# DanieleTeni/Online-Non-Linear-Centroidal-MPC-with-stability-Guarantees-for-Robust-Locomotion-of-Legged-Robots-

Hardware: AMD Instinct MI355X
Metric: centroidal-MPC solves/sec, N=20 horizon (higher is better)
Workload: dtype f64

## Files before the change

### __graft_entry__.py

```python
import os
import sys

ROOT = os.path.dirname(os.path.abspath(__file__))
if ROOT not in sys.path:
    sys.path.insert(0, ROOT)


def build():
    import build as _b
    _b.build_hip()
    _b.build_oracle()
    _b.build_emu()
    _b.build_emu_gain()
    _b.build_emu_consts()
    _b.build_emu_reuse()
    _b.build_emu_reuse(reuse=False)
    _b.build_device_unit()
    _b.build_tools()
    import ctypes
    import torch
    import cmpc_amd
    from cmpc_amd import capi
    lib = ctypes.CDLL(capi.LIB_PATH)
    for sym in capi.SYMBOLS:
        getattr(lib, sym)


def smoke():
    import numpy as np
    import torch
    import cmpc_amd
    from cmpc_amd import workloads as wl
    from cmpc_amd.solver import BatchedCentroidalMPC
    from oracle import oracle_lib as ol

    assert torch.cuda.is_available(), "smoke() needs a GPU"
    spec, rec = wl.make_workload("perturbed", B=8, N=10, scale=0.25)
    solver = BatchedCentroidalMPC(spec, device="cuda:0")
    out, status, iters, kkt = solver.solve(torch.from_numpy(rec).to("cuda:0"))
# ... 18 lines not shown
```

### build.py

```python
import os
import subprocess
import sys

ROOT = os.path.dirname(os.path.abspath(__file__))
PKG = os.path.join(ROOT, "online-non-linear-centroidal-mpc-with-stability-guarantees-for-robust-locomotion-of-legged-robots-_amd")


def _newer(target, sources):
    if not os.path.exists(target):
        return True
    t = os.path.getmtime(target)
    return any(os.path.getmtime(s) > t for s in sources)


CSRC = os.path.join(PKG, "csrc")
KERNEL_DEPS = [os.path.join(CSRC, "cmpc_kernel.hpp"), os.path.join(CSRC, "cmpc_lds_asm.hpp"), os.path.join(CSRC, "cmpc_wave.hpp"),
               os.path.join(ROOT, "include", "cmpc.h")]
DEVICE_DEPS = [os.path.join(CSRC, "cmpc_hip.hip"), os.path.join(CSRC, "wbc_qp.hip")] + KERNEL_DEPS + [
    os.path.join(CSRC, "cmpc_order_fit.h"), os.path.join(ROOT, "include", "cmpc_wbc.h")]
EMU_DIR = os.path.join(ROOT, "tests", "emu")


def _hipcc_lib(out, defines=(), force=False, verbose=False):
    if force or _newer(out, DEVICE_DEPS):
# ... 5 lines not shown

def _emu_lib(src, out, defines=(), force=False):
    src, out = os.path.join(EMU_DIR, src), os.path.join(EMU_DIR, out)
    if force or _newer(out, [src, os.path.join(EMU_DIR, "cmpc_emu.cpp")] + KERNEL_DEPS):
        subprocess.check_call(["g++", "-O2", "-std=c++17", "-mfma", "-ffp-contract=off", "-fPIC", "-shared", "-pthread"]
                              + ["-D" + d for d in defines] + ["-o", out, src])
    return out


def build_hip(force=False, verbose=False):
    return _hipcc_lib(os.path.join(PKG, "libcmpc_amd.so"), force=force, verbose=verbose)


def build_hip_profile(force=False):
    return _hipcc_lib(os.path.join(ROOT, "tools", "libcmpc_amd_prof.so"), ["CMPC_PROFILE"], force)


def build_hip_dev(force=False):
    return _hipcc_lib(os.path.join(ROOT, "tools", "libcmpc_amd_dev.so"), ["CMPC_DEV_KNOBS"], force)


def build_hip_no_reuse(force=False, profile=False):
    return _hipcc_lib(os.path.join(ROOT, "tools", "libcmpc_amd_noreuse_prof.so" if profile else "libcmpc_amd_noreuse.so"),
                      ["CMPC_NO_EVAL_REUSE"] + (["CMPC_PROFILE"] if profile else []), force)


def build_oracle(force=False):
    out = os.path.join(ROOT, "oracle", "libcmpc_oracle.so")
    deps = [os.path.join(ROOT, "oracle", "cmpc_oracle.c"), os.path.join(ROOT, "include", "cmpc.h")]
    if force or _newer(out, deps):
        subprocess.check_call(["make", "-C", os.path.join(ROOT, "oracle"), "-B", "libcmpc_oracle.so"],
                              stdout=subprocess.DEVNULL)
    return out


def build_emu(force=False):
    return _emu_lib("cmpc_emu.cpp", "libcmpc_emu.so", force=force)


def build_emu_gain(force=False):
    return _emu_lib("cmpc_emu_gain.cpp", "libcmpc_emu_gain.so", force=force)


def build_emu_consts(force=False):
    return _emu_lib("cmpc_emu_consts.cpp", "libcmpc_emu_consts.so", force=force)


def build_emu_reuse(force=False, reuse=True):
    return _emu_lib("cmpc_emu_reuse.cpp", "libcmpc_emu_reuse.so" if reuse else "libcmpc_emu_noreuse.so",
                    [] if reuse else ["CMPC_NO_EVAL_REUSE"], force)


def build_device_unit(force=False):
    src = os.path.join(ROOT, "tests", "gpu_unit", "cmpc_device_unit.hip")
    out = os.path.join(ROOT, "tests", "gpu_unit", "libcmpc_device_unit.so")
    if force or _newer(out, [src] + KERNEL_DEPS):
        subprocess.check_call(["hipcc", "--offload-arch=gfx950", "-O3", "-std=c++17", "-fPIC", "-shared", "-o", out, src])
    return out


def build_tools(force=False):
    outs = []
    for name in ("hbm_calib", "lds_b128_repro"):
        src = os.path.join(ROOT, "tools", "ubench", name + ".hip")
        out = os.path.join(ROOT, "tools", "ubench", name)
        if force or _newer(out, [src]):
            r = subprocess.run(["hipcc", "--offload-arch=gfx950", "-O3", "-o", out, src], capture_output=True, text=True)
            if r.returncode != 0:
                print(f"build_tools: {name} failed to compile (profiling scripts that need it will not run)\n{r.stderr}",
                      file=sys.stderr)
                continue
        outs.append(out)
    return outs


if __name__ == "__main__":
    force = "--force" in sys.argv
    print(build_hip(force, verbose="-v" in sys.argv))
    print(build_oracle(force))
    print(build_emu(force))
    print(build_emu_gain(force))
    print(build_emu_consts(force))
    print(build_emu_reuse(force))
    print(build_emu_reuse(force, reuse=False))
    print(build_device_unit(force))
    print(build_tools(force))
```

### online-non-linear-centroidal-mpc-with-stability-guarantees-for-robust-locomotion-of-legged-robots-_amd/csrc/cmpc_kernel.hpp

```cpp
#pragma once
#include "../../include/cmpc.h"
#include <math.h>
#include <utility>
#ifdef CMPC_HOST_EMU
#include <cstdio>
#include <cstdlib>
#endif

#ifndef CMPC_HOST_EMU
#include <hip/hip_runtime.h>
#define CMPC_DEV __device__ __forceinline__
#define CMPC_LANE ((int)threadIdx.x)
#define CMPC_SYNC() asm volatile("s_waitcnt lgkmcnt(0)" ::: "memory")
#define CMPC_SYNC_GLOBAL() __syncthreads()
#define CMPC_SYNC_WG() asm volatile("s_waitcnt lgkmcnt(0)\n\ts_barrier" ::: "memory")
#define CMPC_WAVE_ID() ((int)__builtin_amdgcn_readfirstlane((int)threadIdx.x >> 6))
static __device__ __forceinline__ double cmpc_bcast(double v, int src) {
  union { double d; int i[2]; } u; u.d = v;
  u.i[0] = __builtin_amdgcn_readlane(u.i[0], src);
  u.i[1] = __builtin_amdgcn_readlane(u.i[1], src);
  return u.d;
}
#define CMPC_BCAST(v, src) cmpc_bcast((v), (src))
typedef double cmpc_v4d __attribute__((ext_vector_type(4)));
// ... 11 lines not shown
#else
#define SPD(field) (EVAL_REUSE ? cmpc_fresh(CMPC_SPEC_OR_ROW(field)) : CMPC_SPEC_OR_ROW(field))
#endif
typedef const double __attribute__((address_space(4))) *cmpc_crow_t;
#define CMPC_CROW(p) ((cmpc_crow_t)(p))
static __device__ __forceinline__ cmpc_crow_t cmpc_fresh_row(cmpc_crow_t r) { asm volatile("" : "+s"(r)); return r; }
#define CMPC_ROW_AT(r, i) (cmpc_fresh_row(r)[i])
static __device__ __forceinline__ double cmpc_uniform_d(double v) {
  union { double d; int i[2]; } u; u.d = v;
  int lo, hi;
  asm("s_nop 0\n\tv_readfirstlane_b32 %0, %2\n\tv_readfirstlane_b32 %1, %3\n\ts_nop 1" : "=s"(lo), "=s"(hi) : "v"(u.i[0]), "v"(u.i[1]));
  u.i[0] = lo; u.i[1] = hi;
  return u.d;
}
#ifdef CMPC_NO_UNIFORM_D
#define CMPC_UNIFORM_D(x) (x)
#else
#define CMPC_UNIFORM_D(x) cmpc_uniform_d(x)
#endif
#define CMPC_SCHED_FENCE() __builtin_amdgcn_sched_barrier(0)
#define CMPC_RELANE(x) do { (x) = (int)__builtin_amdgcn_mbcnt_hi(~0u, __builtin_amdgcn_mbcnt_lo(~0u, 0u)) + lane_base; } while (0)
#define CMPC_SYNC_WAVE(w) CMPC_SYNC()
#define CMPC_FENCE_WAVE(w) asm volatile("s_waitcnt vmcnt(0) lgkmcnt(0)" ::: "memory")
#endif
#ifdef CMPC_HOST_EMU
#define CMPC_SYNC_WAVE(w) emu_barrier_wait(&emu_wave_barrier[(w)])
#define CMPC_FENCE_WAVE(w) emu_barrier_wait(&emu_wave_barrier[(w)])
#define CMPC_SYNC_WG() emu_barrier_wait(&emu_barrier)
#endif
#ifndef CMPC_RELANE
#define CMPC_RELANE(x) do { } while (0)
#define SPD(field) CMPC_SPEC_OR_ROW(field)
typedef const double *cmpc_crow_t;
#define CMPC_CROW(p) ((cmpc_crow_t)(p))
#define CMPC_ROW_AT(r, i) ((r)[i])
#define CMPC_FRESH_D(x) (x)
#define CMPC_UNIFORM_D(x) (x)
#endif
#define CMPC_CIDX(field) ((int)((__builtin_offsetof(cmpc_spec, field) - __builtin_offsetof(cmpc_spec, delta)) / sizeof(double)))
#define CMPC_SPEC_OR_ROW(field) (CONSTS ? CMPC_ROW_AT(crow, CMPC_CIDX(field)) : sp.field)
static_assert(CMPC_CIDX(relax) == CMPC_NCONST - 1 && CMPC_CIDX(box[2]) == 13 && __builtin_offsetof(cmpc_spec, tol) == __builtin_offsetof(cmpc_spec, relax) + sizeof(double),
              "the row of per-instance constants is the block of cmpc_spec from delta to relax");
#define CMPC_FMA(x, y, z) __builtin_fma((x), (y), (z))
#ifndef CMPC_OPAQUE_D
#define CMPC_OPAQUE_D(x) do { } while (0)
#endif
#ifndef CMPC_UNIFORM_INT
#define CMPC_UNIFORM_INT(x) (x)
#endif
#ifndef CMPC_OPAQUE_S
#define CMPC_OPAQUE_S(x) do { } while (0)
#endif

#if defined(CMPC_PROFILE) && !defined(CMPC_HOST_EMU)
static __device__ __forceinline__ constexpr int cmpc_retry_class(int slot) {
  return (slot == 11 || slot == 12 || slot == 26 || slot == 0) ? 31
       : (slot == 24 || slot == 25) ? 32
       : (slot == 27) ? 34
       : 33;
}
#define CMPC_TICK(slot) do { long long now_ = clock64(); tprof[slot] += now_ - tlast; \
    if (prof_retry) tprof[cmpc_retry_class(slot)] += now_ - tlast; \
    tlast = now_; } while (0)
#define CMPC_TICK_RESET() do { tlast = clock64(); } while (0)
#define CMPC_RETRY_STAT(slot, n) do { tprof[slot] += (n); } while (0)
#define CMPC_RETRY_MARK(on) do { prof_retry = (on); } while (0)
#define CMPC_RETRY_TRACK 1
#else
#define CMPC_TICK(slot) do { } while (0)
#define CMPC_TICK_RESET() do { } while (0)
#define CMPC_RETRY_MARK(on) do { } while (0)
#define CMPC_RETRY_TRACK 0
#endif
#ifndef CMPC_RETRY_STAT
#define CMPC_RETRY_STAT(slot, n) do { } while (0)
#endif
#define CMPC_NPROF 36

namespace cmpc {

struct KArgs {
  cmpc_spec sp;
  int B;
  const double *recs;
  const double *warm;
  const double *state_in;
  double *state_out;
  double *out;
  int32_t *status;
  int32_t *iters;
  double *kkt;
  double *scratch;
  size_t scratch_stride;
  long long *prof;
  double tol_acc, tol_tenth;
};

enum { R_LYAP = 0, R_CZ = 1, R_HWC = 2, R_BOX = 3, R_FRIC = 15 };
// ... 108 lines not shown
  using S = Sizes<4, 1>;
#ifdef CMPC_NO_GT_FIRST
  static constexpr bool GT = true, GT_FIRST = false;
#else
  static constexpr bool GT = true, GT_FIRST = !PIPE;
#endif
  static constexpr int oM = 0;
  static constexpr int oP = oM + S::NTRI + (S::NTRI & 1);
  static constexpr bool P_PACKED = true;
  static constexpr int P_DOUBLES = S::NPT + (S::NPT & 1);
  static constexpr int DUMPN = 16;
  static constexpr int MISCN = 52;
  static constexpr int oXN1 = oP + P_DOUBLES;
  static constexpr int oSR = oXN1 + S::NXA;
  static constexpr int oSRP = oSR + 20;
  static constexpr int oHDR = oSRP + 20;
  static constexpr int oH0 = oHDR + 24;
  static constexpr int oH1 = oH0 + S::NZ;
  static constexpr int oPC1 = oH1 + S::NZ;
  static constexpr int oPC = oPC1 + S::NXA;
  static constexpr int oRED = oPC + S::NXA;
  static constexpr int oCOLD = oRED + 4;
  static constexpr int oDUMP = oCOLD + 8;
  static constexpr int oXK = oDUMP + DUMPN + ((oDUMP + DUMPN) & 1);
  static constexpr int oUK = oXK + S::NXA;
  static constexpr int oLAMK = oUK + S::NU;
  static constexpr int oLAMN = oLAMK + S::NXA;
  static constexpr int oUPX = oLAMN + S::NXA;
  static constexpr int oSK = oUPX + S::NU;
  static constexpr int oZK = oSK + S::NI;
  static constexpr int oVDV = oZK + S::NI;
  static constexpr int oMISC = oVDV + 3 * S::NF;
  static constexpr int oLATE = oMISC + MISCN;
  static constexpr int LATE_DOUBLES = S::NZ + 4 * S::NI;
  static constexpr int oAL = GT_FIRST ? oP : oLATE;
  static constexpr int oGK = oAL + S::NZ;
  static constexpr int oW0 = oGK + S::NI;
  static constexpr int oW1 = oW0 + S::NI;
  static constexpr int oW2 = oW1 + S::NI;
  static_assert(!GT_FIRST || LATE_DOUBLES <= P_DOUBLES, "the late evaluation vectors fit the dead P region");
  static constexpr int oGH = GT_FIRST ? oM : oLATE + LATE_DOUBLES;
  static constexpr int oBV = oGH + 3 * S::NZ;
  static constexpr int oVR = GT_FIRST ? oBV + S::NXA : oAL;
  static constexpr int oEND = GT_FIRST ? oLATE : oBV + S::NXA;
  static constexpr int oTV = oSK;
  static constexpr int oTV2 = oXK;
// ... 60 lines not shown
    ok = ok && v < INFINITY && v > -INFINITY && (positive ? v > 0.0 : (gain || v >= 0.0));
  }
  return ok;
}

template <int NV, int NW = 1, bool PIPE = false, bool GAIN = false, bool CONSTS = false> struct Solver {
  using D = Dims<NV, NW, PIPE>;
  static constexpr int XCH_DU = 16, XCH_DOUBLES = XCH_DU + 2 * D::NU;
  static_assert(!PIPE || XCH_DOUBLES <= D::P_DOUBLES, "the exchange words fit in the unused P region of the second image");
  static constexpr int XCH_AT = D::LDS_DOUBLES + D::oP;
  static_assert(!PIPE || NW == 1, "the pipelined pair runs the one-wave solver");
  static_assert(!PIPE || (D::oUB + 64 <= D::oBV && D::oUB >= D::oXN1 + D::NXA && !D::GT_FIRST),
                "pair_vectors reads BV / writes XN1 of the image the Riccati wave is working in");
  static constexpr int NF = D::NF, NU = D::NU, NXA = D::NXA, NZ = D::NZ, NI = D::NI, NH = D::NH, WS = D::WS;
  static_assert(NW == 1 || NU <= 64, "the input rows (pivot chains, substitutions) live in the first wave");
#ifdef CMPC_NO_EVAL_REUSE
  static constexpr bool EVAL_REUSE = false;
#else
  static constexpr bool EVAL_REUSE = NV == 4 && NW == 1 && !PIPE && !GAIN && D::GT_FIRST;
#endif
  static constexpr bool RETRY_TRACK_POSSIBLE = NV == 4 && NW == 1 && !PIPE && !GAIN;
  static constexpr int ER_AT = 256;
  static_assert(!RETRY_TRACK_POSSIBLE || (ER_AT >= 3 * NZ + NXA + 3 * NF && ER_AT + 6 * WS <= D::NTRI), "the parked error measures fit the M region");
  static constexpr bool RETRY_TRACK = EVAL_REUSE || (CMPC_RETRY_TRACK && NV == 4 && NW == 1 && !PIPE && !GAIN);

  const KArgs &ka;
  const cmpc_spec &sp;
  double *lds;
  double *ldsR;
  int lane_base = 0;
  GArr gs;
  GArr rec;
  int N, lane;
  int wv = 0;
  GArr gx, glam, gdx, glamn, gu, gdu, gupx, gsl, gz, gds, gdz;
  int lr[NH][6];
  double lg[NH][6];
  double piv_min = PIV_MIN;
  GArr st_in{nullptr};
  long long tprof[CMPC_NPROF] = {0, 0, 0, 0, 0, 0, 0, 0, 0, 0, 0, 0, 0, 0, 0, 0, 0, 0, 0, 0, 0, 0, 0, 0, 0, 0, 0, 0, 0, 0, 0, 0, 0, 0, 0, 0}, tlast = 0;
  bool prof_retry = false;
  double *gain_out = nullptr;
  GArr gbuf{nullptr};
  bool gain_sweep = false;
  cmpc_crow_t crow = nullptr;

  CMPC_DEV Solver(const KArgs &a, double *l, double *g, const double *r)
// ... 28 lines not shown
    else {
#ifdef CMPC_HOST_EMU
      CMPC_SYNC();
#else
      if constexpr (NW == 1) CMPC_SYNC(); else CMPC_SYNC_WG();
#endif
    }
  }
  CMPC_DEV void gsync() const {
    if constexpr (PIPE) { CMPC_FENCE_WAVE(wv); } else { CMPC_SYNC_GLOBAL(); }
  }
  CMPC_DEV void pair_sync() const { if constexpr (PIPE) { CMPC_SYNC_GLOBAL(); } }
  CMPC_DEV bool first_wave() const { return NW == 1 || wv == 0; }

  CMPC_DEV double gam_k(int k, int f) const { return (k == N) ? L(D::oHDR + 22 + f) : L(D::oSR + 17 + f); }
  CMPC_DEV double gam_km1(int f) const { return L(D::oSRP + 17 + f); }
  CMPC_DEV void vert_local(int j, double &vx, double &vy) const {
    const double Lh = SPD(foot_length) * 0.5, Wh = SPD(foot_width) * 0.5;
    const double cx[8] = {Lh, Lh, -Lh, -Lh, Lh, 0.0, -Lh, 0.0};
    const double cy[8] = {Wh, -Wh, -Wh, Wh, 0.0, -Wh, 0.0, Wh};
    vx = cx[j]; vy = cy[j];
  }

  CMPC_DEV void load_stage(int k) {
    static_assert(NXA <= 64 && NU <= 64, "one lane per state / input component");
    constexpr int NIH = (NI + WS - 1) / WS;
    const bool in = k < N;
    const int kn = in ? k + 1 : k, ku = in ? k : N - 1, kp = (k >= 1) ? k - 1 : 0;
    const int ix = (lane < NXA) ? lane : 0, iu = (lane < NU) ? lane : 0, ir = (lane < 19) ? lane : 0;
    const double x0 = gx[k * NXA + ix], x1 = gx[kn * NXA + ix];
    const double u0 = gu[ku * NU + iu], up = gupx[ku * NU + iu];
    const double r0 = rec[24 + 19 * ku + ir], r1 = rec[24 + 19 * kp + ir], hd = rec[(lane < 24) ? lane : 0];
    double sv[NIH], zv[NIH];
    const double l0 = glam[k * NXA + ix], l1 = glam[kn * NXA + ix];
    {
#pragma unroll
      for (int h = 0; h < NIH; ++h) {
        const int r = lane + WS * h, rc = (r < NI) ? r : 0;
        sv[h] = gsl[k * NI + rc]; zv[h] = gz[k * NI + rc];
      }
    }
    if (lane < NXA) {
      L(D::oXK + lane) = x0; L(D::oXN1 + lane) = in ? x1 : 0.0;
      L(D::oLAMK + lane) = l0; L(D::oLAMN + lane) = in ? l1 : 0.0;
    }
    if (lane < NU) { L(D::oUK + lane) = in ? u0 : 0.0; L(D::oUPX + lane) = in ? up : 0.0; }
    {
#pragma unroll
      for (int h = 0; h < NIH; ++h) {
        const int r = lane + WS * h;
        if (r < NI) { L(D::oSK + r) = sv[h]; L(D::oZK + r) = zv[h]; }
      }
    }
    if (lane < 19) { L(D::oSR + lane) = in ? r0 : 0.0; L(D::oSRP + lane) = (k >= 1) ? r1 : 0.0; }
    if (lane < 24) L(D::oHDR + lane) = hd;
    sync();
  }

  CMPC_DEV void stage_geometry(int k) {
    const double d = SPD(delta), m = L(D::oHDR + 20);
    double *tq = &L(D::oH0), *yw = &L(D::oH0 + 3 * NF), *qq = &L(D::oH0 + 6 * NF);
    static_assert(7 * NF <= 2 * NZ, "vertex products fit the H0/H1 block");
    if (lane < NF) {
      const int f = lane / NV, j = lane % NV;
      const double yaw = L(D::oXK + 12 + 4 * f);
      const double px = L(D::oXK + 13 + 4 * f), py = L(D::oXK + 14 + 4 * f), pz = L(D::oXK + 15 + 4 * f);
      const double cx = L(D::oXK + 0), cy = L(D::oXK + 1), cz = L(D::oXK + 2);
      const double fx = L(D::oUK + 3 * lane), fy = L(D::oUK + 3 * lane + 1), fz = L(D::oUK + 3 * lane + 2);
      const double p0 = d * L(D::oLAMN + 6), p1 = d * L(D::oLAMN + 7), p2 = d * L(D::oLAMN + 8);
      const double cs = cos(yaw), sn = sin(yaw);
      double vx, vy; vert_local(j, vx, vy);
      const double rvx = cs * vx - sn * vy, rvy = sn * vx + cs * vy;
      const double dvx = -sn * vx - cs * vy, dvy = cs * vx - sn * vy;
      const double rx = px + rvx - cx, ry = py + rvy - cy, rz = pz - cz;
      L(D::oVDV + 3 * lane + 0) = dvx; L(D::oVDV + 3 * lane + 1) = dvy; L(D::oVDV + 3 * lane + 2) = 0.0;
      L(D::oVR + 3 * lane + 0) = rx; L(D::oVR + 3 * lane + 1) = ry; L(D::oVR + 3 * lane + 2) = rz;
      tq[3 * lane + 0] = ry * fz - rz * fy; tq[3 * lane + 1] = rz * fx - rx * fz; tq[3 * lane + 2] = rx * fy - ry * fx;
      yw[3 * lane + 0] = dvy * fz; yw[3 * lane + 1] = -dvx * fz; yw[3 * lane + 2] = dvx * fy - dvy * fx;
      qq[lane] = p0 * (-rvy * fz) + p1 * (rvx * fz) + p2 * (-rvx * fy + rvy * fx);
// ... 893 lines not shown
      const double a = (b0 + b1) + (b2 + b3);
      L(D::oXN1 + lane) = R(D::oPC + lane) + a;
      st[D::gB + lane] = L(D::oBV + lane);
    }
  }
  CMPC_DEV double list_dot(int h, const double *v) const {
    double a = 0.0;
#pragma unroll
    for (int n = 0; n < 6; ++n) a = CMPC_FMA(lg[h][n], v[lr[h][n]], a);
    CMPC_OPAQUE_D(a);
    return a;
  }

  CMPC_DEV void eval_stage(int k, double mu, double reg, double wz, double x0n2, Err &er, bool init, bool reuse_ = false) {
    const bool reuse = EVAL_REUSE && reuse_;
    CMPC_RELANE(lane); CMPC_OPAQUE(lane);
    if constexpr (EVAL_REUSE) { CMPC_OPAQUE_S(k); }
    double re_h0 = 0.0, re_h1 = 0.0, re_al = 0.0, re_w0 = 0.0;
    if (reuse) {
      const GArr sk = stage(k); const unsigned re = restage(k);
      const int cz = (lane < NZ) ? lane : 0, ci = (lane < NI) ? lane : 0;
      re_al = sk[D::gAL + cz]; re_w0 = sk[re + D::rW0 + ci]; re_h0 = sk[re + D::rH0 + cz]; re_h1 = sk[re + D::rH1 + cz];
    }
    load_stage(k);
    CMPC_TICK(24);
    const GArr st = stage(k);
    if (reuse) {
      const unsigned re = restage(k);
      const int cz = (lane < NZ) ? lane : 0, cx = (lane < NXA) ? lane : 0, ci = (lane < NI) ? lane : 0;
      static_assert(!EVAL_REUSE || (NH == 1 && NI <= WS && 3 * NF + 5 <= WS && D::rQ == D::rVDV + 3 * NF && D::rPI == D::rQ + 2), "one word of each kept vector per lane");
      const double re_gh0 = st[D::gGH + cz], re_gh1 = st[D::gGH + D::GHS + cz], re_gh2 = st[D::gGH + 2 * D::GHS + cz];
      const double re_bv = st[D::gB + cx];
      const double re_vdv = st[re + D::rVDV + ((lane < 3 * NF + 5) ? lane : 0)];
      const int dump = D::oDUMP + (lane & (D::DUMPN - 1));
      const bool in_z = lane < NZ;
      L(in_z ? D::oGH + lane : dump) = re_gh0; L(in_z ? D::oGH + NZ + lane : dump) = re_gh1; L(in_z ? D::oGH + 2 * NZ + lane : dump) = re_gh2;
      L((lane < NXA) ? D::oBV + lane : dump) = (k < N) ? re_bv : 0.0;
      L((lane < 3 * NF) ? D::oVDV + lane : (lane < 3 * NF + 2) ? D::oMISC + 30 - 3 * NF + lane
        : (lane < 3 * NF + 5) ? D::oMISC + 9 - (3 * NF + 2) + lane : dump) = re_vdv;
      static_assert(!EVAL_REUSE || (D::oLAMK == D::oUK + NU && NU + NXA == NZ), "the Lyapunov gradient fits the inputs and lam_k");
      L(in_z ? D::oUK + lane : dump) = re_al; L(in_z ? D::oH0 + lane : dump) = re_h0; L(in_z ? D::oH1 + lane : dump) = re_h1;
      L((lane < NI) ? D::oSK + lane : dump) = re_w0;
      sync();
      CMPC_RETRY_STAT(30, 1);
      CMPC_TICK(27);
    } else if (k < N) {
      stage_geometry(k);
// ... 208 lines not shown
    }
    sync();
  }

  CMPC_DEV bool matrix_sweep(double mu, double reg, double x0n2, Err &er, bool init, int &k_done) {
    const bool retry = RETRY_TRACK && k_done <= N;
    er.e_d = er.e_p = er.e_c = er.e_cmu = er.sum_mult = 0.0; er.n_mult = 0;
    if (retry) {
      const double *w = &L(D::oM + ER_AT + 6 * lane);
      er.e_d = w[0]; er.e_p = w[1]; er.e_c = w[2]; er.e_cmu = w[3]; er.sum_mult = w[4]; er.n_mult = (int)w[5];
      CMPC_RETRY_STAT(28, 1);
    }
    piv_min = fmax(PIV_MIN, PIV_FRAC * reg);
    const double e1 = 2.718281828459045235360287;
    double ez = CMPC_UNIFORM_D(exp(-(double)(N - 1)));
    CMPC_OPAQUE_D(ez);
    if constexpr (!PIPE) {
      for (int k = N; k >= 0; --k) {
        const double wz = SPD(w_cz_const) * 0.5 * ez + SPD(w_cz_const) * 0.5;
        ez *= e1;
        if constexpr (RETRY_TRACK) {
          const bool done = k >= k_done;
          CMPC_RETRY_MARK(done);
          if (EVAL_REUSE || !done) eval_stage(k, mu, reg, wz, x0n2, er, init, done);
          else { Err again = er; eval_stage(k, mu, reg, wz, x0n2, again, init); }
          if (!riccati_stage(k)) {
            CMPC_RETRY_MARK(false);
            if (!init) { CMPC_RETRY_STAT(29, N + 1 - k); if (k < k_done) k_done = CMPC_UNIFORM_INT(k); }
            if (retry) CMPC_RETRY_STAT(35, 1);
            if (!init) {
              double *w = &L(D::oM + ER_AT + 6 * lane);
              w[0] = er.e_d; w[1] = er.e_p; w[2] = er.e_c; w[3] = er.e_cmu; w[4] = er.sum_mult; w[5] = (double)er.n_mult;
            }
            return false;
          }
          CMPC_RETRY_MARK(false);
        } else {
          eval_stage(k, mu, reg, wz, x0n2, er, init);
          if (!riccati_stage(k)) return false;
        }
      }
      return true;
    } else {
      double *xch = ldsR + XCH_AT;
      if (lane == 0 && wv == 0) { xch[8] = 0.0; xch[9] = 0.0; }
      CMPC_SYNC_WG();
      for (int j = 0; j <= N + 2; ++j) {
        if (wv == 1) {
// ... 319 lines not shown
    }
    ap = red_min(lap); ad = red_min(lad);
    if (lane == 0) { xch[6] = ap; xch[7] = ad; }
    CMPC_SYNC_WG();
  }

  CMPC_DEV double jg_dot(int r, double lyap_dot, const double *dx, const double *du, double hw0, double hw1, double hw2,
                         double g0, double g1, double muf) const {
    const bool is_box = r >= R_BOX && r < R_FRIC, is_fr = r >= R_FRIC;
    const int qb = is_box ? r - R_BOX : 0, fb = qb / 6, ab = (qb % 6) / 2;
    const int qf = is_fr ? r - R_FRIC : 0, v = qf / 5, t = qf % 5;
    const double d2 = dx[2], d6 = dx[6], d7 = dx[7], d8 = dx[8], dbx = dx[13 + 4 * fb + ab];
    const double fx = du[3 * v], fy = du[3 * v + 1], fz = du[3 * v + 2];
    const int sgn = (qb & 1) ? -1 : 1;
    const double v_box = sgn * (fb ? g1 : g0) * dbx;
    const double gg = (v / NV) ? g1 : g0;
    const double v_fr = (t == 0) ? gg * (fx - muf * fz) : (t == 1) ? gg * (-fx - muf * fz) : (t == 2) ? gg * (fy - muf * fz)
                      : (t == 3) ? gg * (-fy - muf * fz) : -gg * fz;
    const double v_hw = 2.0 * (hw0 * d6 + hw1 * d7 + hw2 * d8);
    return (r == R_LYAP) ? lyap_dot : (r == R_CZ) ? d2 : (r == R_HWC) ? v_hw : (is_box ? v_box : v_fr);
  }

  CMPC_DEV void apply_step(double mu, double ap, double ad) {
    gsync();
    constexpr int UF = 4;
    const bool do_xu = !PIPE || wv == 0, do_sz = !PIPE || wv == 1;
    if (do_xu)
    for (int e0 = NXA; e0 < (N + 1) * NXA; e0 += WS * UF) {
      double a[UF], b[UF], c[UF], d[UF];
#pragma unroll
      for (int q = 0; q < UF; ++q) {
        const int e = e0 + lane + WS * q, ec = (e < (N + 1) * NXA) ? e : NXA;
        a[q] = gx[ec]; b[q] = gdx[ec]; c[q] = glam[ec]; d[q] = glamn[ec];
      }
#pragma unroll
      for (int q = 0; q < UF; ++q) {
        const int e = e0 + lane + WS * q;
        if (e < (N + 1) * NXA) { gx[e] = a[q] + ap * b[q]; glam[e] = c[q] + ap * (d[q] - c[q]); }
      }
    }
    if (do_xu)
    for (int e0 = 0; e0 < N * NU; e0 += WS * UF) {
      double a[UF], b[UF];
#pragma unroll
      for (int q = 0; q < UF; ++q) {
        const int e = e0 + lane + WS * q, ec = (e < N * NU) ? e : 0;
        a[q] = gu[ec]; b[q] = gdu[ec];
      }
#pragma unroll
      for (int q = 0; q < UF; ++q) {
        const int e = e0 + lane + WS * q;
        if (e < N * NU) gu[e] = a[q] + ap * b[q];
      }
    }
    if (do_sz)
    for (int e0 = 0; e0 < (N + 1) * NI; e0 += WS * UF) {
      double zq[UF], sq[UF], dsq[UF], dzq[UF];
#pragma unroll
      for (int q = 0; q < UF; ++q) {
        const int e = e0 + lane + WS * q, ec = (e < (N + 1) * NI) ? e : 0;
        zq[q] = gz[ec]; sq[q] = gsl[ec]; dsq[q] = gds[ec]; dzq[q] = gdz[ec];
      }
#pragma unroll
      for (int q = 0; q < UF; ++q) {
        const int e = e0 + lane + WS * q;
        if (e < (N + 1) * NI && zq[q] != 0.0) {
          const double s = sq[q] + ap * dsq[q];
          const double z = zq[q] + ad * dzq[q];
          const double lo = mu / s / 1e10, hi = mu / s * 1e10;
          gsl[e] = s; gz[e] = fmin(fmax(z, lo), hi);
        }
      }
    }
    gsync();
  }

  CMPC_DEV void initial_point(const double *warm_, const double *prox_, bool resume) {
    const GArr warm{const_cast<double *>(warm_)}, prox{const_cast<double *>(prox_)};
    const bool has_warm = warm_ != nullptr, has_prox = prox_ != nullptr;
    const double m = rec[20];
    double *srct = &L(D::oM);
    for (int k = lane; k <= N; k += WS) {
      int src = k;
      if (resume) {
        const double gl = rec[(k < N) ? 24 + 19 * k + 17 : 22], gr = rec[(k < N) ? 24 + 19 * k + 18 : 23];
        const int kn = (k < N) ? k + 1 : N;
        const bool same = gl == st_in[D::state_fl(N) + k] && gr == st_in[D::state_fl(N) + N + 1 + k];
        const bool next = k < N && gl == st_in[D::state_fl(N) + kn] && gr == st_in[D::state_fl(N) + N + 1 + kn];
        if (!same && next) src = k + 1;
      }
      srct[k] = (double)src;
    }
    sync();
    for (int e = lane; e < (N + 1) * NXA; e += WS) {
      const int k = e / NXA, i = e % NXA, ks = (int)srct[k];
      double v = 0.0;
// ... 209 lines not shown
    bool ret_saved = false;
    double kkt = INFINITY;
    for (;;) {
    if (state_out && lane == 0) GArr{state_out}[D::state_mu(N)] = 0.0;
    double mu = resume ? st_in[D::state_mu(N)] : MU_INIT;
    kkt = INFINITY; st = CMPC_MAX_ITER;
    constexpr bool CNT_LDS = (NW == 1);
    int n_acc = 0, n_stall = 0, polish = -1, since_best = 0;
    constexpr int SAVED = 256;
    constexpr int NOSTEP = 512;
    double &reg_last = R(D::oCOLD + 0), &kkt_best = R(D::oCOLD + 1), &kkt_saved = R(D::oCOLD + 2);
    double &snapped = R(D::oCOLD + 3);
    {
      double inf = INFINITY, zero = 0.0;
      CMPC_OPAQUE_D(inf); CMPC_OPAQUE_D(zero);
      const double ks0 = kkt_saved;
      if constexpr (PIPE) { CMPC_SYNC_WG(); } else sync();
      double at0 = sp.acc_tol;
      CMPC_OPAQUE_D(at0);
      const bool carry = spent > 0 && ks0 <= fmax(at0, tol_());
      reg_last = zero; kkt_best = inf; snapped = zero;
      if (!carry) kkt_saved = inf;
      if constexpr (CNT_LDS) { R(D::oCOLD + 4) = zero; R(D::oCOLD + 5) = zero; R(D::oCOLD + 6) = zero - 1.0; R(D::oCOLD + 7) = zero; }
    }
    auto acc_raw = [&]() { double a = sp.acc_tol; CMPC_OPAQUE_D(a); return a; };
    auto acc_tol = [&]() { return fmax(acc_raw(), tol_()); };
    auto save_tol = [&]() { return fmax(fmax(acc_raw(), tol_()), tol_acc); };
    if (!PIPE || wv == 0) initial_point(resume ? state_in : warm, warm, resume);
    pair_sync();
    CMPC_TICK_RESET();
    for (it = 0; it <= sp.max_iter - spent; ++it) {
      double reg = 0.0;
      Err er;
      bool fail = false;
      const double mu_sweep = mu;
      const double rl = reg_last;
      int k_done = N + 1;
#ifdef CMPC_TEST_FAIL_ITER
      if (!resume && it == (CMPC_TEST_FAIL_ITER)) fail = true; else
#endif
      while (!matrix_sweep(mu, reg, x0n2, er, it == 0, k_done)) {
        if constexpr (EVAL_REUSE) gsync(); else sync();
        if (reg == 0.0) reg = (rl == 0.0) ? 1e-4 : fmax(1e-20, rl / 3);
        else reg *= (rl == 0.0) ? 100.0 : 8.0;
        if (reg > 1e20) { fail = true; break; }
      }
      if (fail) { st = CMPC_NUMERICAL | NOSTEP; break; }
#ifdef CMPC_DEBUG_FIRST_SWEEP
      if (it == 0) break;
#endif
      double e_d = red_max(er.e_d), e_p = red_max(er.e_p), e_c = red_max(er.e_c), e_cmu = red_max(er.e_cmu);
      double sm = red_sum(er.sum_mult), nm = red_sum((double)er.n_mult);
      if constexpr (PIPE) {
        double *xch = ldsR + XCH_AT;
        if (wv == 1 && lane == 0) { xch[0] = e_d; xch[1] = e_p; xch[2] = e_c; xch[3] = e_cmu; xch[4] = sm; xch[5] = nm; }
        pair_sync();
        e_d = xch[0]; e_p = xch[1]; e_c = xch[2]; e_cmu = xch[3]; sm = xch[4]; nm = xch[5];
      }
      const double sd = fmax(100.0, sm / fmax(nm, 1.0)) / 100.0;
      kkt = fmax(fmax(e_d / sd, e_p), e_c / sd);
#ifdef CMPC_HOST_EMU
      if (lane == 0 && getenv("CMPC_EMU_TRACE"))
        printf("it %3d d=%.2e p=%.2e c=%.2e mu=%.1e reg=%.1e\n", it, e_d / sd, e_p, e_c / sd, mu, reg);
#endif
      const double ebar = fmax(fmax(e_d / sd, e_p), e_cmu / sd);
      double ks = kkt_saved, kb = kkt_best;
      const bool unsnapped = snapped == 0.0;
      if constexpr (CNT_LDS) {
        n_acc = (int)R(D::oCOLD + 4); since_best = (int)R(D::oCOLD + 5); polish = (int)R(D::oCOLD + 6); n_stall = (int)R(D::oCOLD + 7);
      }
      if constexpr (PIPE) { CMPC_SYNC_WG(); } else sync();
      if (polish >= 0 && kkt > tol_acc) {
        st = CMPC_CONVERGED | SAVED; kkt = ks; break;
      }
      if (polish < 0) {
        if (kkt <= save_tol() && kkt < ks) {
          if (!PIPE || wv == 0) write_solution(out);
          if constexpr (GAIN) { if (!PIPE || wv == 0) write_state(gbuf.p, mu); }
          ks = kkt; kkt_saved = kkt;
        }
        if (kkt <= tol_()) {
          if (state_out && mu >= MU_WARM && unsnapped) { if (!PIPE || wv == 0) write_state(state_out, mu); snapped = 1.0; }
          polish = POLISH_ITERS; mu = tol_10;
        } else {
          n_acc = (kkt <= tol_acc) ? n_acc + 1 : 0;
          if (n_acc >= ACC_ITERS) { st = CMPC_ACCEPTABLE | SAVED; kkt = ks; break; }
          {
            const double kw = (mu <= tol_10) ? kkt : ebar;
            if (kw < 0.5 * kb) { kb = kw; kkt_best = kw; since_best = 0; } else ++since_best;
            if (since_best >= NOPROG_ITERS && ks <= acc_tol()) {
              st = CMPC_ACCEPTABLE | SAVED; kkt = ks; break;
            }
          }
        }
      }
      if (polish == 0) {
        st = CMPC_CONVERGED;
        if (kkt > tol_() && kkt > ks) { kkt = ks; st = CMPC_CONVERGED | SAVED; }
        break;
// ... 19 lines not shown
          CMPC_OPAQUE_D(inf);
          kkt_best = inf; since_best = 0;
        }
        if (state_out && mu_before >= MU_WARM && mu < MU_WARM && unsnapped) { if (!PIPE || wv == 0) write_state(state_out, mu_before); snapped = 1.0; }
      }
      if constexpr (CNT_LDS) { R(D::oCOLD + 4) = (double)n_acc; R(D::oCOLD + 5) = (double)since_best; R(D::oCOLD + 6) = (double)polish; }
      double ap, ad;
      auto count_stall = [&]() {
        if constexpr (CNT_LDS) {
          const int ns = (int)R(D::oCOLD + 7);
          if constexpr (PIPE) { CMPC_SYNC_WG(); } else sync();
          R(D::oCOLD + 7) = (ap < STALL_STEP) ? (double)(ns + 1) : 0.0;
        } else n_stall = (ap < STALL_STEP) ? n_stall + 1 : 0;
      };
      if constexpr (PIPE) {
        vector_sweeps(mu, mu - mu_sweep, ap, ad);
        count_stall();
        apply_step(mu, ap, ad);
        pair_sync();
      } else {
        vector_sweeps(mu, mu - mu_sweep, ap, ad);
        CMPC_TICK(6);
        count_stall();
        apply_step(mu, ap, ad);
        CMPC_TICK(7);
      }
    }
    bool use_saved = (st & SAVED) != 0;
    const bool nostep = (st & NOSTEP) != 0;
    st &= SAVED - 1;
    const double ks_end = kkt_saved;
    if (nostep && ks_end <= acc_tol()) { st = CMPC_ACCEPTABLE; kkt = ks_end; use_saved = true; }
    const bool keep = resume && (st == CMPC_MAX_ITER || st == CMPC_NUMERICAL) && ks_end <= acc_tol();
    if (keep && !(it < sp.max_iter)) { st = CMPC_ACCEPTABLE; kkt = ks_end; use_saved = true; }
    if (!use_saved && !keep && (!PIPE || wv == 0)) write_solution(out);
    if constexpr (GAIN) ret_saved = use_saved;
    const int again = CMPC_UNIFORM_INT((int)(resume && (st == CMPC_MAX_ITER || st == CMPC_NUMERICAL) && it < sp.max_iter));
    if (!again) break;
    spent = CMPC_UNIFORM_INT(spent + it); resume = false;
    if constexpr (PIPE) pair_sync(); else gsync();
    }
    if (lane == 0 && (!PIPE || wv == 0)) {
      *status = st; *iters = it + spent; *kkt_out = kkt;
      if (state_out) GArr{state_out}[D::state_mu(N) + 1] = (double)(it + spent);
    }
    if constexpr (GAIN) gain_tail(st, ret_saved, warm);
#if defined(CMPC_PROFILE) && !defined(CMPC_HOST_EMU)
    if (lane == 0 && ka.prof)
      for (int i = 0; i < CMPC_NPROF; ++i) atomicAdd((unsigned long long *)&ka.prof[i], (unsigned long long)tprof[i]);
#endif
    if constexpr (PIPE) pair_sync(); else sync();
  }
};

template <int NV, int NW, bool PIPE, bool GAIN, bool CONSTS>
CMPC_DEV void run_instance(const KArgs &ka, double *lds, double *slab, int p, unsigned slot, double *gain, double *gbuf,
                           const double *consts) {
// ... 20 lines not shown
```

Measured before the change: 90010.

## Fuse the primal-dual step update into the next iteration's stage loads

Instead of a separate apply_step pass that sweeps all x, u, lambda, slack and dual arrays after each iteration, the step lengths are parked in LDS. The next iteration's load_stage applies the update per stage as it loads, then writes the updated values back. A finish_step path applies any pending update on failure, and extra global syncs are added before solution writes. This removes one full global read/write sweep and its barriers per iteration, at the cost of more complex control flow and extra loads in the stage-load path.

```diff
diff --git a/__graft_entry__.py b/__graft_entry__.py
--- a/__graft_entry__.py
+++ b/__graft_entry__.py
@@ -15,6 +15,8 @@
     _b.build_emu_consts()
     _b.build_emu_reuse()
     _b.build_emu_reuse(reuse=False)
+    _b.build_emu_step()
+    _b.build_emu_step(fused=False)
     _b.build_device_unit()
     _b.build_tools()
     import ctypes
diff --git a/build.py b/build.py
--- a/build.py
+++ b/build.py
@@ -51,7 +51,12 @@
 
 def build_hip_no_reuse(force=False, profile=False):
     return _hipcc_lib(os.path.join(ROOT, "tools", "libcmpc_amd_noreuse_prof.so" if profile else "libcmpc_amd_noreuse.so"),
-                      ["CMPC_NO_EVAL_REUSE"] + (["CMPC_PROFILE"] if profile else []), force)
+                      ["CMPC_NO_EVAL_REUSE", "CMPC_SEPARATE_STEP"] + (["CMPC_PROFILE"] if profile else []), force)
+
+
+def build_hip_separate_step(force=False, profile=False):
+    return _hipcc_lib(os.path.join(ROOT, "tools", "libcmpc_amd_sepstep_prof.so" if profile else "libcmpc_amd_sepstep.so"),
+                      ["CMPC_SEPARATE_STEP"] + (["CMPC_PROFILE"] if profile else []), force)
 
 
 def build_oracle(force=False):
@@ -78,6 +83,11 @@
 def build_emu_reuse(force=False, reuse=True):
     return _emu_lib("cmpc_emu_reuse.cpp", "libcmpc_emu_reuse.so" if reuse else "libcmpc_emu_noreuse.so",
                     [] if reuse else ["CMPC_NO_EVAL_REUSE"], force)
+
+
+def build_emu_step(force=False, fused=True):
+    return _emu_lib("cmpc_emu_step.cpp", "libcmpc_emu_step.so" if fused else "libcmpc_emu_sepstep.so",
+                    [] if fused else ["CMPC_SEPARATE_STEP"], force)
 
 
 def build_device_unit(force=False):
@@ -112,5 +122,7 @@
     print(build_emu_consts(force))
     print(build_emu_reuse(force))
     print(build_emu_reuse(force, reuse=False))
+    print(build_emu_step(force))
+    print(build_emu_step(force, fused=False))
     print(build_device_unit(force))
     print(build_tools(force))
diff --git a/online-non-linear-centroidal-mpc-with-stability-guarantees-for-robust-locomotion-of-legged-robots-_amd/csrc/cmpc_kernel.hpp b/online-non-linear-centroidal-mpc-with-stability-guarantees-for-robust-locomotion-of-legged-robots-_amd/csrc/cmpc_kernel.hpp
--- a/online-non-linear-centroidal-mpc-with-stability-guarantees-for-robust-locomotion-of-legged-robots-_amd/csrc/cmpc_kernel.hpp
+++ b/online-non-linear-centroidal-mpc-with-stability-guarantees-for-robust-locomotion-of-legged-robots-_amd/csrc/cmpc_kernel.hpp
@@ -57,11 +57,15 @@
 #define CMPC_RELANE(x) do { (x) = (int)__builtin_amdgcn_mbcnt_hi(~0u, __builtin_amdgcn_mbcnt_lo(~0u, 0u)) + lane_base; } while (0)
 #define CMPC_SYNC_WAVE(w) CMPC_SYNC()
 #define CMPC_FENCE_WAVE(w) asm volatile("s_waitcnt vmcnt(0) lgkmcnt(0)" ::: "memory")
+#define CMPC_VM_LANDED() __builtin_amdgcn_s_waitcnt(0x0F70)
+#define CMPC_ASM_NOTE(text) asm volatile("; " text)
 #endif
 #ifdef CMPC_HOST_EMU
 #define CMPC_SYNC_WAVE(w) emu_barrier_wait(&emu_wave_barrier[(w)])
 #define CMPC_FENCE_WAVE(w) emu_barrier_wait(&emu_wave_barrier[(w)])
 #define CMPC_SYNC_WG() emu_barrier_wait(&emu_barrier)
+#define CMPC_VM_LANDED() do { } while (0)
+#define CMPC_ASM_NOTE(text) do { } while (0)
 #endif
 #ifndef CMPC_RELANE
 #define CMPC_RELANE(x) do { } while (0)
@@ -77,6 +81,11 @@
 static_assert(CMPC_CIDX(relax) == CMPC_NCONST - 1 && CMPC_CIDX(box[2]) == 13 && __builtin_offsetof(cmpc_spec, tol) == __builtin_offsetof(cmpc_spec, relax) + sizeof(double),
               "the row of per-instance constants is the block of cmpc_spec from delta to relax");
 #define CMPC_FMA(x, y, z) __builtin_fma((x), (y), (z))
+#ifdef CMPC_HOST_EMU
+#define CMPC_STEP_MAD(t, b, a) ((a) + (t) * (b))
+#else
+#define CMPC_STEP_MAD(t, b, a) __builtin_fma((t), (b), (a))
+#endif
 #ifndef CMPC_OPAQUE_D
 #define CMPC_OPAQUE_D(x) do { } while (0)
 #endif
@@ -109,6 +118,9 @@
 #endif
 #ifndef CMPC_RETRY_STAT
 #define CMPC_RETRY_STAT(slot, n) do { } while (0)
+#endif
+#ifndef CMPC_STEP_STAT
+#define CMPC_STEP_STAT(slot, n) do { } while (0)
 #endif
 #define CMPC_NPROF 36
 
@@ -263,6 +275,7 @@
   static constexpr int oRED = oPC + S::NXA;
   static constexpr int oCOLD = oRED + 4;
   static constexpr int oDUMP = oCOLD + 8;
+  static constexpr int oSTEP_AP = oSR + 19, oSTEP_AD = oSRP + 19, oSTEP_ON = oRED + 3;
   static constexpr int oXK = oDUMP + DUMPN + ((oDUMP + DUMPN) & 1);
   static constexpr int oUK = oXK + S::NXA;
   static constexpr int oLAMK = oUK + S::NU;
@@ -369,7 +382,12 @@
   static constexpr bool RETRY_TRACK_POSSIBLE = NV == 4 && NW == 1 && !PIPE && !GAIN;
   static constexpr int ER_AT = 256;
   static_assert(!RETRY_TRACK_POSSIBLE || (ER_AT >= 3 * NZ + NXA + 3 * NF && ER_AT + 6 * WS <= D::NTRI), "the parked error measures fit the M region");
-  static constexpr bool RETRY_TRACK = EVAL_REUSE || (CMPC_RETRY_TRACK && NV == 4 && NW == 1 && !PIPE && !GAIN);
+#ifdef CMPC_SEPARATE_STEP
+  static constexpr bool STEP_FUSED = false;
+#else
+  static constexpr bool STEP_FUSED = RETRY_TRACK_POSSIBLE;
+#endif
+  static constexpr bool RETRY_TRACK = EVAL_REUSE || STEP_FUSED || (CMPC_RETRY_TRACK && NV == 4 && NW == 1 && !PIPE && !GAIN);
 
   const KArgs &ka;
   const cmpc_spec &sp;
@@ -444,17 +462,44 @@
     vx = cx[j]; vy = cy[j];
   }
 
-  CMPC_DEV void load_stage(int k) {
+  CMPC_DEV static double step_axpy(double a, double t, double b) { return CMPC_STEP_MAD(t, b, a); }
+  CMPC_DEV static double step_toward(double c, double t, double d) { return CMPC_STEP_MAD(t, d - c, c); }
+  CMPC_DEV static void step_slack(double &s, double &z, double ds, double dz, double ap, double ad, double mu) {
+    s = CMPC_STEP_MAD(ap, ds, s);
+    const double zn = CMPC_STEP_MAD(ad, dz, z);
+    const double lo = mu / s / 1e10, hi = mu / s * 1e10;
+    z = fmin(fmax(zn, lo), hi);
+  }
+
+  CMPC_DEV void load_stage(int k, bool first = false, double mu = 0.0) {
     static_assert(NXA <= 64 && NU <= 64, "one lane per state / input component");
     constexpr int NIH = (NI + WS - 1) / WS;
     const bool in = k < N;
     const int kn = in ? k + 1 : k, ku = in ? k : N - 1, kp = (k >= 1) ? k - 1 : 0;
     const int ix = (lane < NXA) ? lane : 0, iu = (lane < NU) ? lane : 0, ir = (lane < 19) ? lane : 0;
-    const double x0 = gx[k * NXA + ix], x1 = gx[kn * NXA + ix];
-    const double u0 = gu[ku * NU + iu], up = gupx[ku * NU + iu];
+    bool step = false;
+    if constexpr (STEP_FUSED) { if (first) step = CMPC_UNIFORM_INT((int)(L(D::oSTEP_ON) != 0.0)) != 0; }
+    double dxv = 0.0, lnv = 0.0, duv = 0.0, dsv[NIH], dzv[NIH];
+#pragma unroll
+    for (int h = 0; h < NIH; ++h) { dsv[h] = 0.0; dzv[h] = 0.0; }
+    if constexpr (STEP_FUSED) {
+      if (step) {
+        dxv = gdx[k * NXA + ix]; lnv = glamn[k * NXA + ix]; duv = gdu[ku * NU + iu];
+#pragma unroll
+        for (int h = 0; h < NIH; ++h) {
+          const int r = lane + WS * h, rc = (r < NI) ? r : 0;
+          dsv[h] = gds[k * NI + rc]; dzv[h] = gdz[k * NI + rc];
+        }
+      }
+    }
+    double x0 = gx[k * NXA + ix];
+    const double x1 = gx[kn * NXA + ix];
+    double u0 = gu[ku * NU + iu];
+    const double up = gupx[ku * NU + iu];
     const double r0 = rec[24 + 19 * ku + ir], r1 = rec[24 + 19 * kp + ir], hd = rec[(lane < 24) ? lane : 0];
     double sv[NIH], zv[NIH];
-    const double l0 = glam[k * NXA + ix], l1 = glam[kn * NXA + ix];
+    double l0 = glam[k * NXA + ix];
+    const double l1 = glam[kn * NXA + ix];
     {
 #pragma unroll
       for (int h = 0; h < NIH; ++h) {
@@ -462,6 +507,21 @@
         sv[h] = gsl[k * NI + rc]; zv[h] = gz[k * NI + rc];
       }
     }
+    if constexpr (STEP_FUSED) {
+      if (step) {
+        const double ap = L(D::oSTEP_AP), ad = L(D::oSTEP_AD);
+        if (k >= 1) { x0 = step_axpy(x0, ap, dxv); l0 = step_toward(l0, ap, lnv); }
+        if (in) u0 = step_axpy(u0, ap, duv);
+#pragma unroll
+        for (int h = 0; h < NIH; ++h) {
+          double sn = sv[h], zn = zv[h];
+          step_slack(sn, zn, dsv[h], dzv[h], ap, ad, mu);
+          const bool on = zv[h] != 0.0;
+          sv[h] = on ? sn : sv[h]; zv[h] = on ? zn : zv[h];
+        }
+        CMPC_STEP_STAT(0, 1);
+      }
+    }
     if (lane < NXA) {
       L(D::oXK + lane) = x0; L(D::oXN1 + lane) = in ? x1 : 0.0;
       L(D::oLAMK + lane) = l0; L(D::oLAMN + lane) = in ? l1 : 0.0;
@@ -477,6 +537,19 @@
     if (lane < 19) { L(D::oSR + lane) = in ? r0 : 0.0; L(D::oSRP + lane) = (k >= 1) ? r1 : 0.0; }
     if (lane < 24) L(D::oHDR + lane) = hd;
     sync();
+    if constexpr (STEP_FUSED) {
+      CMPC_VM_LANDED();
+      if (step) {
+        CMPC_ASM_NOTE("cmpc: the step's stores");
+        if (k >= 1 && lane < NXA) { gx[k * NXA + lane] = x0; glam[k * NXA + lane] = l0; }
+        if (in && lane < NU) gu[k * NU + lane] = u0;
+#pragma unroll
+        for (int h = 0; h < NIH; ++h) {
+          const int r = lane + WS * h;
+          if (r < NI) { gsl[k * NI + r] = sv[h]; gz[k * NI + r] = zv[h]; }
+        }
+      }
+    }
   }
 
   CMPC_DEV void stage_geometry(int k) {
@@ -1416,7 +1489,7 @@
       const int cz = (lane < NZ) ? lane : 0, ci = (lane < NI) ? lane : 0;
       re_al = sk[D::gAL + cz]; re_w0 = sk[re + D::rW0 + ci]; re_h0 = sk[re + D::rH0 + cz]; re_h1 = sk[re + D::rH1 + cz];
     }
-    load_stage(k);
+    load_stage(k, !reuse_, mu);
     CMPC_TICK(24);
     const GArr st = stage(k);
     if (reuse) {
@@ -1671,8 +1744,11 @@
         if constexpr (RETRY_TRACK) {
           const bool done = k >= k_done;
           CMPC_RETRY_MARK(done);
-          if (EVAL_REUSE || !done) eval_stage(k, mu, reg, wz, x0n2, er, init, done);
-          else { Err again = er; eval_stage(k, mu, reg, wz, x0n2, again, init); }
+          if constexpr (EVAL_REUSE) eval_stage(k, mu, reg, wz, x0n2, er, init, done);
+          else {
+            Err again = er;
+            eval_stage(k, mu, reg, wz, x0n2, done ? again : er, init, done);
+          }
           if (!riccati_stage(k)) {
             CMPC_RETRY_MARK(false);
             if (!init) { CMPC_RETRY_STAT(29, N + 1 - k); if (k < k_done) k_done = CMPC_UNIFORM_INT(k); }
@@ -2038,6 +2114,7 @@
   }
 
   CMPC_DEV void apply_step(double mu, double ap, double ad) {
+    CMPC_STEP_STAT(1, 1);
     gsync();
     constexpr int UF = 4;
     const bool do_xu = !PIPE || wv == 0, do_sz = !PIPE || wv == 1;
@@ -2052,7 +2129,7 @@
 #pragma unroll
       for (int q = 0; q < UF; ++q) {
         const int e = e0 + lane + WS * q;
-        if (e < (N + 1) * NXA) { gx[e] = a[q] + ap * b[q]; glam[e] = c[q] + ap * (d[q] - c[q]); }
+        if (e < (N + 1) * NXA) { gx[e] = step_axpy(a[q], ap, b[q]); glam[e] = step_toward(c[q], ap, d[q]); }
       }
     }
     if (do_xu)
@@ -2066,7 +2143,7 @@
 #pragma unroll
       for (int q = 0; q < UF; ++q) {
         const int e = e0 + lane + WS * q;
-        if (e < N * NU) gu[e] = a[q] + ap * b[q];
+        if (e < N * NU) gu[e] = step_axpy(a[q], ap, b[q]);
       }
     }
     if (do_sz)
@@ -2081,13 +2158,18 @@
       for (int q = 0; q < UF; ++q) {
         const int e = e0 + lane + WS * q;
         if (e < (N + 1) * NI && zq[q] != 0.0) {
-          const double s = sq[q] + ap * dsq[q];
-          const double z = zq[q] + ad * dzq[q];
-          const double lo = mu / s / 1e10, hi = mu / s * 1e10;
-          gsl[e] = s; gz[e] = fmin(fmax(z, lo), hi);
-        }
-      }
-    }
+          double s = sq[q], z = zq[q];
+          step_slack(s, z, dsq[q], dzq[q], ap, ad, mu);
+          gsl[e] = s; gz[e] = z;
+        }
+      }
+    }
+    gsync();
+  }
+
+  CMPC_DEV void finish_step(double mu, int k_done) {
+    if (CMPC_UNIFORM_INT((int)(L(D::oSTEP_ON) != 0.0)) == 0) return;
+    for (int k = k_done - 1; k >= 0; --k) { load_stage(k, true, mu); CMPC_STEP_STAT(2, 1); }
     gsync();
   }
 
@@ -2343,6 +2425,7 @@
       reg_last = zero; kkt_best = inf; snapped = zero;
       if (!carry) kkt_saved = inf;
       if constexpr (CNT_LDS) { R(D::oCOLD + 4) = zero; R(D::oCOLD + 5) = zero; R(D::oCOLD + 6) = zero - 1.0; R(D::oCOLD + 7) = zero; }
+      if constexpr (STEP_FUSED) L(D::oSTEP_ON) = zero;
     }
     auto acc_raw = [&]() { double a = sp.acc_tol; CMPC_OPAQUE_D(a); return a; };
     auto acc_tol = [&]() { return fmax(acc_raw(), tol_()); };
@@ -2366,7 +2449,11 @@
         else reg *= (rl == 0.0) ? 100.0 : 8.0;
         if (reg > 1e20) { fail = true; break; }
       }
-      if (fail) { st = CMPC_NUMERICAL | NOSTEP; break; }
+      if (fail) {
+        if constexpr (STEP_FUSED) finish_step(mu, k_done);
+        st = CMPC_NUMERICAL | NOSTEP; break;
+      }
+      if constexpr (STEP_FUSED) L(D::oSTEP_ON) = 0.0;
 #ifdef CMPC_DEBUG_FIRST_SWEEP
       if (it == 0) break;
 #endif
@@ -2396,6 +2483,7 @@
       }
       if (polish < 0) {
         if (kkt <= save_tol() && kkt < ks) {
+          if constexpr (STEP_FUSED) gsync();
           if (!PIPE || wv == 0) write_solution(out);
           if constexpr (GAIN) { if (!PIPE || wv == 0) write_state(gbuf.p, mu); }
           ks = kkt; kkt_saved = kkt;
@@ -2461,8 +2549,12 @@
         vector_sweeps(mu, mu - mu_sweep, ap, ad);
         CMPC_TICK(6);
         count_stall();
-        apply_step(mu, ap, ad);
-        CMPC_TICK(7);
+        if constexpr (STEP_FUSED) {
+          L(D::oSTEP_AP) = ap; L(D::oSTEP_AD) = ad; L(D::oSTEP_ON) = 1.0;
+        } else {
+          apply_step(mu, ap, ad);
+          CMPC_TICK(7);
+        }
       }
     }
     bool use_saved = (st & SAVED) != 0;
@@ -2472,6 +2564,7 @@
     if (nostep && ks_end <= acc_tol()) { st = CMPC_ACCEPTABLE; kkt = ks_end; use_saved = true; }
     const bool keep = resume && (st == CMPC_MAX_ITER || st == CMPC_NUMERICAL) && ks_end <= acc_tol();
     if (keep && !(it < sp.max_iter)) { st = CMPC_ACCEPTABLE; kkt = ks_end; use_saved = true; }
+    if constexpr (STEP_FUSED) { if (!use_saved && !keep) gsync(); }
     if (!use_saved && !keep && (!PIPE || wv == 0)) write_solution(out);
     if constexpr (GAIN) ret_saved = use_saved;
     const int again = CMPC_UNIFORM_INT((int)(resume && (st == CMPC_MAX_ITER || st == CMPC_NUMERICAL) && it < sp.max_iter));
```

New measurement: 91920, median of 6. 2.1% higher.
